# leejet/stable-diffusion.cpp

Hardware: AMD Instinct MI355X
Metric: denoise it/s (image-iterations/s: cond+uncond UNet forwards per image per step) (higher is better)
Workload: dtype f16; 1 GPU; sd15 UNet 512x512, cfg 7 (cond+uncond), f16 weights, batch 8/GPU, Euler-A step; global_batch=8, flash_attn=True, hip_graph=1, cfg_pair_in_one_graph=True, device_resident_sampler=True

## Files before the change

### stable-diffusion.cpp_amd/csrc/backend/planner.cpp

```cpp
#include "planner.h"

#include <atomic>
#include <cstddef>
#include <cstdio>
#include <cstdlib>
#include <cstring>
#include <functional>
#include <memory>
#include <mutex>
#include <string>
#include <algorithm>
#include <map>
#include <unordered_map>
#include <unordered_set>
#include <vector>

#include "kernels.h"
#include "ktime.h"

namespace mi355x {

static uint8_t g_opmap[256];
static uint8_t g_unmap[256];
static bool g_opmap_init = [] {
// ... 4268 lines not shown

namespace {
struct OptionRow {
    const char* key;
    std::atomic<int> Options::*member;
    void (*setter)(int);
};
#define OPT(name) {#name, &Options::name, nullptr}
const OptionRow g_option_table[] = {
    OPT(fusion),
    OPT(mfma_gemm),
    OPT(hip_graph),
    OPT(flash_pattern),
    {"gemm16_t320", nullptr, gemm16_set_t320},
    {"t256p_pad", nullptr, gemm16_set_t256p_pad},
    {"tail_split", nullptr, gemm16_set_tail_split},
    {"conv_wmajor", nullptr, gemm16_set_conv_wmajor},
    {"ln16_rows", nullptr, gemm16_set_ln16_rows},
    {"t320_linear_max_split", nullptr, gemm16_set_t320_linear_max_split},
    OPT(qgemv),
    OPT(fuse_q16),
    {"streamk", nullptr, gemm16_set_streamk},
    {"geglu16", nullptr, gemm16_set_geglu16},
    {"bn64_max_tiles", nullptr, gemm16_set_bn64_max},
    {"conv3w_prio", nullptr, conv3w_set_prio},
    {"t256p_min_nt_sk", nullptr, gemm16_set_t256p_min_nt_sk},
    {"t256p_min_tiles_sk", nullptr, gemm16_set_t256p_min_tiles_sk},
    {"conv3w", nullptr, conv3w_set},
    OPT(hoist_emb),
    OPT(fuse_rows16),
    OPT(fuse_cat_rows16),
    OPT(fuse_gn_stats),
    OPT(fuse_gn_epilogue),
    OPT(fuse_tile_merge),
    OPT(fuse_model_input),
    OPT(fuse_guidance3),
    OPT(fuse_patch_embed),
    OPT(fuse_ip_attn),
    OPT(fuse_joint_qkv),
    OPT(fuse_ln_reduce),
    OPT(jit_qimages),
    {"qinloop_min_rows", nullptr, gemm16_set_qinloop_min_rows},
    OPT(fuse_flash_slices),
    {"gemm16_t192p", nullptr, gemm16_set_t192p},
    {"conv3w_min_blocks", nullptr, conv3w_set_min_blocks},
    {"conv3w_min_blocks_deep", nullptr, conv3w_set_min_blocks_deep},
// ... 63 lines not shown
```

### stable-diffusion.cpp_amd/csrc/kernels/conv3w.hip

```cpp
#include <cstdio>
#include <cstdlib>

#include "device_utils.h"
#include "g16_common.h"
#include "kernels.h"
#include "ktime.h"

namespace mi355x {

template <int TW, int BN>
struct C3Geom {
    static constexpr int TR     = 256 / TW;
    static constexpr int PITCH  = TW + 16;
    static constexpr int WROWS  = TR + 2;
    static constexpr int WBYTES = WROWS * PITCH * 64;
    static constexpr int NWP    = WBYTES / 1024;
    static constexpr int NWPW   = (NWP + 7) / 8;
    static constexpr int WBUF   = NWPW * 8 * 1024;
    static constexpr int CB     = BN / 64;
    static constexpr int NF     = (BN / 32) * 2;
    static constexpr int BSTAGE = NF * 1024;
    static constexpr int NST    = 4;
    static constexpr int LDS    = 2 * WBUF + NST * BSTAGE;
    static constexpr int RB1    = TW >= 64 ? 32 * 64 : (32 / TW) * PITCH * 64;
    static_assert(WBYTES % 1024 == 0 && PITCH % 16 == 0 && NWPW <= 5 && LDS <= 160 * 1024, "window geometry");
};

#define C3_RD(DST_, ADDR_, OFF_) asm volatile("ds_read_b128 %0, %1 offset:%2" : "=v"(DST_) : "v"(ADDR_), "n"(OFF_))
#define C3_TIE(X_) asm volatile("" : "+v"(X_))

template <int TW, int BN, int PRIO = 3>
__global__ __launch_bounds__(512, 2) void k_conv3w(G16Args g) {
    using G = C3Geom<TW, BN>;
    constexpr int CB = G::CB, CL = CB - 2, PITCH = G::PITCH, NWPW = G::NWPW, WBUF = G::WBUF, BSTAGE = G::BSTAGE, NF = G::NF, RB1 = G::RB1;
    static_assert(CB >= 3, "at least three column blocks per wave");
    __shared__ __attribute__((aligned(1024))) char smem[G::LDS];

    const int lane = threadIdx.x & 63;
    const int wave = __builtin_amdgcn_readfirstlane(threadIdx.x >> 6);
    const int wr = wave & 3, wc = wave >> 2;
    const int hi = lane >> 5;
    if constexpr (PRIO == 3) {
        if (wave >= 4) __builtin_amdgcn_s_setprio(1);
    }

    int bid, kslice;
    g16_wg_order(g, g.ncol_tiles, bid, kslice);
    const int row_tile = bid / g.ncol_tiles;
    const int col_tile = bid - row_tile * g.ncol_tiles;
    const int64_t row0 = (int64_t)row_tile * 256;
    const int col0     = col_tile * BN;

    int icb0 = 0, nicb = g.nt;
    if (g.split_k > 1) {
        icb0 = kslice * g.nt_slice;
        nicb = min(g.nt_slice, g.nt - icb0);
        g.dst += (int64_t)kslice * g.slab;
    }
// ... 180 lines not shown
        C3_RD(BL[0], bcur, (0 * 2) * 1024);                                                                                  \
        C3_RD(BL[1], bcur, (1 * 2) * 1024);                                                                                  \
        if constexpr (CL > 2) C3_RD(BL[CL - 1], bcur, (2 * 2) * 1024);                                                       \
        C3_RD(BH0[0], bcur, ((CB - 2) * 2) * 1024);                                                                          \
        C3_RD(BH0[1], bcur, ((CB - 1) * 2) * 1024);                                                                          \
        for (int ib_ = 0; ib_ + 1 < nicb; ++ib_) C3_BLOCK(NP_, false);                                                       \
        C3_BLOCK(NP_, true);                                                                                                 \
        asm volatile("s_waitcnt lgkmcnt(0)" ::: "memory");                                                                   \
    } while (0)

    if constexpr (NF % 8 != 0) {
        if (w_short)
            C3_MAIN(NPBMAX - 1);
        else
            C3_MAIN(NPBMAX);
    } else {
        C3_MAIN(NPBMAX);
    }

    if (g.ep.gn_rec) {
        static_assert(4 * BN * (int)sizeof(GnRec) <= WBUF, "the tile's records fit one window buffer");
        GnRec* lds = (GnRec*)(smem + (wb ^ 1) * WBUF);
        if (g.ep.residual)
            epi_conv_gn<true, BN, 4, 2, CB>(acc, g, row0, col0, wr, wc, lane, lds);
        else
            epi_conv_gn<false, BN, 4, 2, CB>(acc, g, row0, col0, wr, wc, lane, lds);
        return;
    }
    if (g.ep.residual)
        epi_conv<1>(acc, g, row0, col0, wr, wc, lane);
    else
        epi_conv<0>(acc, g, row0, col0, wr, wc, lane);
}

static int g_conv3w_prio = 3;
void conv3w_set_prio(int v) { g_conv3w_prio = v; }
static int g_conv3w = 1;
void conv3w_set(int v) { g_conv3w = v; }
static int g_conv3w_min_blocks = 8, g_conv3w_min_blocks_deep = 5;
void conv3w_set_min_blocks(int v) { g_conv3w_min_blocks = v > 0 ? v : 1; }
void conv3w_set_min_blocks_deep(int v) { g_conv3w_min_blocks_deep = v > 0 ? v : 1; }

int conv3w_plan(int64_t W, int64_t H, int64_t IC, int64_t N, int64_t OC, int ksize, int stride, bool upscale2x, int* bn_out) {
    if (!g_conv3w || ksize != 3 || stride != 1 || upscale2x) return 0;
    if (!(W == 16 || W == 32 || W == 64 || W == 128) || (H * W) % 256 != 0 || IC < 64) return 0;
    if (N * H * W * ((IC + 63) / 64 * 64) * 2 >= (1ll << 32)) return 0;
    const int bn = OC % 320 == 0 ? 320 : (OC % 256 == 0 ? 256 : 0);
    if (!bn) return 0;
    const int64_t tiles = (H * W * N / 256) * (OC / bn);
    const int64_t nicb  = (IC + 63) / 64 * 2;
// ... 39 lines not shown
    }
    if (e.act >= 0) {
        fprintf(stderr, "ggml-mi355x: conv3w has no fused activation\n");
        abort();
    }
    G16Args g{};
    g.A    = (const _Float16*)x16_nhwc;
    g.W    = (const half8_t*)wswz32;
    g.ICp  = (int)((IC + 63) / 64 * 64);
    g.kfr  = (int64_t)g.ICp * 9 / 16;
    g.dst  = dst;
    g.H    = (int)H;
    g.Wd   = (int)W;
    g.OW   = (int)W;
    g.OH   = (int)H;
    g.OHOW = W * H;
    g.S    = 1;
    g.pad  = 1;
    g.KS   = 3;
    g.nt   = g.ICp / 32;
    g.R    = g.OHOW * N;
    g.C    = OC;
    g.zero = gemm16_zero_page();
    g.ep   = G16Epi{e.bias, e.residual, e.scale};
    g.ep.chan_add = e.chan_add;
    g.ep.chan_ld  = (int)e.chan_ld;
    g.ncol_tiles  = (int)(OC / bn);
    if (e.gn_rec) {
        if ((S > 1 && splitk_ws) || !conv3w_gn_rec_supported(g.OHOW, OC, N)) {
            fprintf(stderr, "ggml-mi355x: conv3w asked for a GroupNorm side band on a launch it does not serve (split %d, %lld positions per image)\n", S, (long long)g.OHOW);
            abort();
        }
        g.ep.gn_rec = e.gn_rec;
    }
    if (S > 1 && splitk_ws) {
        g.split_k  = S;
        g.nt_slice = (g.nt + S - 1) / S;
        g.slab     = g.R * OC;
        g.dst      = splitk_ws;
        g.ep       = G16Epi{nullptr, nullptr, e.scale};
    } else {
        S = 1;
    }
    const unsigned tiles = (unsigned)((g.R / 256) * g.ncol_tiles);
    g.worder             = gemm16_worder_rows(g, tiles, (unsigned)S);
    const double bytes   = (double)N * H * W * g.ICp * 2.0 + (double)g.ICp * 9 * ((OC + 127) / 128 * 128) * 2.0 + (double)g.R * OC * 4.0 * (e.residual ? 2.0 : 1.0);
// ... 19 lines not shown
```

### stable-diffusion.cpp_amd/csrc/kernels/g16_common.h

```cpp
#pragma once
#include "device_utils.h"
#include "kernels.h"

namespace mi355x {

struct G16Epi {
    const float* bias;
    const float* residual;
    float scale;
    const float* gate = nullptr;
    int gate_L        = 0;
    int gelu          = 0;
    const float* chan_add = nullptr;
    int chan_ld           = 0;
    GnRec* gn_rec         = nullptr;
};

__device__ __forceinline__ void gn_merge(float& m, float& q, float m2, float q2, float hn) {
    const float d = m2 - m;
    q             = (q + q2) + (d * d) * hn;
    m             = 0.5f * (m + m2);
}
template <int CTRL>
__device__ __forceinline__ float gn_dpp(float v) { return __int_as_float(__builtin_amdgcn_update_dpp(0, __float_as_int(v), CTRL, 0xf, 0xf, true)); }
// ... 55 lines not shown
    int a_runL, a_runS;
    int qt;
    int64_t qrow_bytes;
    int wblk_lim;
    int nt;
    int ncol_tiles;
    int split_k;
    int nt_slice;
    int64_t slab;
    float* sk_slab;
    int* sk_cnt;
    int sk_grid, sk_tiles, sk_dp;
    int split_col;
    _Float16* split_dst16;
    int64_t split_ldd16;
    int multi;
    const half8_t* Wm[16];
    float* dstm[16];
    _Float16* dst16m[16];
    const float* biasm[16];
    int H, Wd, ICp, OH, OW, S, pad, UPS, KS, icb_per_tap, tap_major;
    int64_t OHOW;
    const _Float16* zero;
    G16Epi ep;
#ifdef MI355X_EXPERIMENTS
    int abl;
#endif
};

int gemm16_worder_rows(const G16Args& g, unsigned gx, unsigned ny);
void gemm16_set_conv_wmajor(int v);
__device__ __forceinline__ void g16_wg_order(const G16Args& g, int ncol_all, int& bid, int& kslice) {
    if (g.worder > 0) {
        const int L  = (int)blockIdx.y * (int)gridDim.x + (int)blockIdx.x;
        const int k  = L & 7, j = L >> 3;
        const int pl = j / g.worder, r = j - pl * g.worder;
        const int p  = pl * 8 + k;
        kslice       = p / ncol_all;
        bid          = r * ncol_all + (p - kslice * ncol_all);
        return;
    }
    const int nb = gridDim.x;
    bid          = blockIdx.x;
    if ((nb & 7) == 0) bid = (bid & 7) * (nb >> 3) + (bid >> 3);
    kslice = blockIdx.y;
}

#define GLDS16(gptr, ldsptr) \
    __builtin_amdgcn_global_load_lds((const __attribute__((address_space(1))) void*)(gptr), (__attribute__((address_space(3))) void*)(ldsptr), 16, 0, 0)


template <typename T>
__device__ __forceinline__ void st_u(T* ubase, uint32_t lane_bytes, T v) { *(T*)((char*)ubase + lane_bytes) = v; }
template <typename T>
// ... 169 lines not shown
                    const int64_t uo  = ub + (int64_t)ro * g.hm_d;
                    const uint32_t lo = le + (ro >= wrap_at ? adj : 0u);
                    const float v     = acc[rb][cb][r] * g.ep.scale + bias;
                    if (MODE == EPI_HM_F32)
                        st_u(g.dst + uo, lo * 4u, v);
                    else
                        st_u(g.dst16 + uo, lo * 2u, (_Float16)v);
                }
            } else {
#pragma unroll
                for (int r = 0; r < 16; ++r) {
                    const int64_t row = base_row + (r & 3) + 8 * (r >> 2) + 4 * hi;
                    if (row >= g.R) continue;
                    float v = acc[rb][cb][r] * g.ep.scale + bias;
                    if (g.ep.residual) v += g.ep.residual[row * g.ldd + col];
                    if (g.dst) g.dst[row * g.ldd + col] = v;
                    if (g.dst16) g.dst16[row * g.ldd16 + col] = (_Float16)v;
                }
            }
        }
    }
}

template <int BM, int RB, int CB>
__device__ __forceinline__ void epi_dispatch_linear(const float16_t (&acc)[RB][CB], const G16Args& g, int64_t row0, int col0, int wr, int wc, int lane) {
    const bool full = row0 + BM <= g.R;
    if (g.geglu_inner > 0 && g.geglu16) {
        epi_geglu16(acc, g, row0, col0, wr, wc, lane);
    } else if (CB % 2 == 0 && g.geglu_inner > 0) {
        if constexpr (CB % 2 == 0) epi_geglu(acc, g, row0, col0, wr, wc, lane);
    } else if (g.hm_d > 0 && g.hm_L >= 32 && !g.ep.residual && (g.dst != nullptr) != (g.dst16 != nullptr)) {
        if (g.dst16)
            epi_linear<EPI_HM_F16>(acc, g, row0, col0, wr, wc, lane);
        else
            epi_linear<EPI_HM_F32>(acc, g, row0, col0, wr, wc, lane);
    } else if (g.ep.gate) {
        epi_linear<EPI_F32_GATE>(acc, g, row0, col0, wr, wc, lane);
    } else if (full && g.hm_d == 0 && g.dst && !g.dst16) {
        if (g.ep.residual)
            epi_linear<EPI_F32_RES>(acc, g, row0, col0, wr, wc, lane);
        else
            epi_linear<EPI_F32>(acc, g, row0, col0, wr, wc, lane);
    } else if (g.hm_d == 0 && g.dst16 && !g.dst && g.ep.residual && !g.ep.gelu) {
        epi_linear<EPI_F16_RES>(acc, g, row0, col0, wr, wc, lane);
    } else if (g.hm_d == 0 && g.dst16 && !g.dst && !g.ep.residual) {
        if (g.ep.gelu)
            epi_linear<EPI_F16_GELU>(acc, g, row0, col0, wr, wc, lane);
        else
            epi_linear<EPI_F16>(acc, g, row0, col0, wr, wc, lane);
// ... 29 lines not shown
            const float* pc  = g.ep.chan_add ? g.ep.chan_add + (int64_t)img0 * cld + cblk : nullptr;
#pragma unroll
            for (int r0 = 0; r0 < 16; r0 += 8) {
                float bv[8], rv[8];
#pragma unroll
                for (int r = r0; r < r0 + 8; ++r) {
                    const int ro  = (r & 3) + 8 * (r >> 2);
                    const bool ok = MODE != 2 || cblk + ro + 4 * hi < g.C;
                    bv[r - r0]    = (pb && ok) ? ld_u(pb + ro, 16u * hi) : 0.f;
                    if (pc && ok) bv[r - r0] += ld_u(pc + ro, (4u * hi + dimg * cld) * 4u);
                    rv[r - r0]    = ((MODE == 1 || (MODE == 2 && g.ep.residual)) && ok) ? ld_u(g.ep.residual + ub + (int64_t)ro * g.OHOW, le * 4u) : 0.f;
                }
#pragma unroll
                for (int r = r0; r < r0 + 8; ++r) {
                    const int ro = (r & 3) + 8 * (r >> 2);
                    if (MODE == 2 && cblk + ro + 4 * hi >= g.C) continue;
                    st_u(g.dst + ub + (int64_t)ro * g.OHOW, le * 4u, acc[rb][cb][r] * g.ep.scale + bv[r - r0] + rv[r - r0]);
                }
            }
        }
    }
}

template <bool RES, int BN, int WR, int RB, int CB>
__device__ __forceinline__ void epi_conv_gn(const float16_t (&acc)[RB][CB], const G16Args& g, int64_t row0, int col0, int wr, int wc, int lane, GnRec* lds) {
    static_assert(WR * RB == 8 && (RB == 1 || RB == 2), "a 256-position tile");
    const int hi = lane >> 5, lc = lane & 31;
    const uint32_t ohow = (uint32_t)g.OHOW;
    const uint32_t img0 = (uint32_t)(row0 / g.OHOW), p0 = (uint32_t)(row0 - (int64_t)img0 * g.OHOW);
    const uint32_t le   = (uint32_t)(wr * (RB * 32) + lc) + 4u * hi * ohow;
    const uint32_t cld  = g.ep.chan_ld ? (uint32_t)g.ep.chan_ld : (uint32_t)g.C;
    const int chl = gn_lane_chan(lane);
#pragma unroll
    for (int cb = 0; cb < CB; ++cb) {
        const int cblk   = col0 + (wc * CB + cb) * 32;
        const int64_t ub = ((int64_t)img0 * g.C + cblk) * g.OHOW + p0;
        const float* pb  = g.ep.bias ? g.ep.bias + cblk : nullptr;
        const float* pc  = g.ep.chan_add ? g.ep.chan_add + (int64_t)img0 * cld + cblk : nullptr;
        float v[RB][16];
#pragma unroll
        for (int r0 = 0; r0 < 16; r0 += 8) {
            float bv[8], rv[RB][8];
#pragma unroll
            for (int r = r0; r < r0 + 8; ++r) {
                const int ro = (r & 3) + 8 * (r >> 2);
                bv[r - r0]   = pb ? ld_u(pb + ro, 16u * hi) : 0.f;
                if (pc) bv[r - r0] += ld_u(pc + ro, 16u * hi);
#pragma unroll
                for (int rb = 0; rb < RB; ++rb) rv[rb][r - r0] = RES ? ld_u(g.ep.residual + ub + (int64_t)ro * g.OHOW + rb * 32, le * 4u) : 0.f;
            }
#pragma unroll
            for (int r = r0; r < r0 + 8; ++r) {
                const int ro = (r & 3) + 8 * (r >> 2);
#pragma unroll
                for (int rb = 0; rb < RB; ++rb) {
                    v[rb][r] = acc[rb][cb][r] * g.ep.scale + bv[r - r0] + rv[rb][r - r0];
                    st_u(g.dst + ub + (int64_t)ro * g.OHOW + rb * 32, le * 4u, v[rb][r]);
                }
            }
        }
        float m, q;
        gn_wave_stats<RB>(v, lane, m, q);
        if (!(lane & 1)) lds[wr * BN + (wc * CB + cb) * 32 + chl] = GnRec{m, q};
    }
    __syncthreads();
    const int c = (wc * WR + wr) * 64 + lane;
    if (c < BN) {
        GnRec a[WR];
#pragma unroll
        for (int i = 0; i < WR; ++i) a[i] = lds[i * BN + c];
        float hn = 16.f * RB;
#pragma unroll
        for (int st = 1; st < WR; st *= 2, hn *= 2.f)
#pragma unroll
            for (int i = 0; i < WR; i += 2 * st) gn_merge(a[i].mean, a[i].m2, a[i + st].mean, a[i + st].m2, hn);
        const uint32_t chunks = ohow / (uint32_t)GN_REC_CHUNK, t = p0 / (uint32_t)GN_REC_CHUNK;
        g.ep.gn_rec[((int64_t)img0 * chunks + t) * g.C + col0 + c] = a[0];
    }
}

}
```

### stable-diffusion.cpp_amd/csrc/kernels/gemm16.hip

```cpp
#include <atomic>
#include <cstdio>
#include <cstdlib>
#include <mutex>
#include <type_traits>
#include <utility>
#include <vector>
#include "device_utils.h"
#include "kernels.h"
#include "ktime.h"
#include "g16_common.h"

namespace mi355x {

template <int BM, int BN, bool CONV, int BK, int NST, int WR, int WC, int PIPE = 0, bool SK = false, int QT = 0>
__global__ __launch_bounds__(WR * WC * 64, PIPE ? 2 : 2) void k_gemm16(G16Args g) {
    static_assert(!SK || (PIPE == 1 && !CONV), "stream-K is written for the pipelined Linear tiles");
    static_assert(QT == 0 || ((QT == 8 || QT == 4) && PIPE == 1 && !CONV && !SK && BM == 256 && (BN == 256 || BN == 192) && WR * WC == 8), "in-loop dequantisation: pipelined 256 x 256 / 256 x 192 Linear tiles");
    constexpr int NW  = WR * WC;
    constexpr int RB  = BM / WR / 32;
    constexpr int CB  = BN / WC / 32;
    static_assert(RB * WR * 32 == BM && CB * WC * 32 == BN, "tile must split into 32x32 blocks per wave");
    constexpr int ROWB   = BK * 2;
    constexpr int SLOTS  = ROWB / 16;
    constexpr int RPP    = 1024 / ROWB;
// ... 2 lines not shown
    constexpr int NF     = (BN / 32) * KSTEPS;
    constexpr int APW    = (ABYTES / 1024) / NW;
    constexpr int WPW    = (NF + NW - 1) / NW;
    constexpr int WEXTRA = NF % NW;
    constexpr int BBYTES = NF * 1024;
    constexpr int NPT    = APW + WPW;
    static_assert(APW * NW * 1024 == ABYTES && APW >= 1, "A stage must split evenly over the waves");
    constexpr int QBLK  = QT == 8 ? 34 : 18;
    constexpr int QPB   = QT == 8 ? 64 : 32;
    constexpr int QNP   = QPB / 16;
    constexpr int QTOFF = 2 * QBLK - 16;
    constexpr int QVC   = 256;
    constexpr int QRAWB = QVC * (QPB + 16);
    constexpr int QNRAW = 3;
    constexpr int QPI   = QT ? QVC * QNP / (NW * 64) : 0;
    constexpr int QRQ   = QPI + 1;
    constexpr int QB0   = NST * ABYTES;
    constexpr int QR0   = QB0 + 2 * BBYTES;
    constexpr int SMEMB = QT ? QR0 + QNRAW * QRAWB : NST * (ABYTES + BBYTES);
    static_assert(SMEMB <= 160 * 1024, "LDS budget");
    __shared__ __attribute__((aligned(1024))) char smem[SMEMB];
    constexpr bool G16_GN_REC_TILE = CONV && BM == 256 && BN != 128 && ((WR == 4 && RB == 2) || (WR == 8 && RB == 1));
    static_assert(!G16_GN_REC_TILE || WR * BN * (int)sizeof(GnRec) <= SMEMB, "the tile's records fit the staging ring");

    const int lane0 = threadIdx.x & 63;
    const int wave = __builtin_amdgcn_readfirstlane(threadIdx.x >> 6);
    const int wr = wave % WR, wc = wave / WR;

    int64_t sk_u = 0, sk_end = 0;
    int sk_w = 0;
    int dp_t = 0, dp_end = 0;
    if constexpr (SK) {
        const int64_t U = (int64_t)(g.sk_tiles - g.sk_dp) * g.nt;
        sk_w            = (g.sk_grid & 7) == 0 ? (int)(blockIdx.x & 7) * (g.sk_grid >> 3) + (int)(blockIdx.x >> 3) : (int)blockIdx.x;
        sk_u            = (int64_t)sk_w * U / g.sk_grid;
        sk_end          = (int64_t)(sk_w + 1) * U / g.sk_grid;
        const int per   = g.sk_dp / g.sk_grid;
        dp_t            = sk_w * per;
        dp_end          = dp_t + per;
    }
  for (bool sk_more = true; sk_more;) {
    int lane = lane0;
    if constexpr (SK) asm volatile("" : "+v"(lane));
    int bid = blockIdx.x, kslice = blockIdx.y;
    int kt0 = 0, nt = g.nt;
    if constexpr (SK) {
// ... 773 lines not shown
                for (int rb = 0; rb < RB; ++rb)
#pragma unroll
                    for (int cb = 0; cb < CB; ++cb)
#pragma unroll
                        for (int i4 = 0; i4 < 4; ++i4) {
                            const u32x4_t v = __builtin_amdgcn_raw_buffer_load_b128(rp, ((((wave * RB + rb) * CB + cb) * 4 + i4) * 64 + lane) * 16, 0, 16);
                            acc[rb][cb][4 * i4] += __uint_as_float(v[0]);
                            acc[rb][cb][4 * i4 + 1] += __uint_as_float(v[1]);
                            acc[rb][cb][4 * i4 + 2] += __uint_as_float(v[2]);
                            acc[rb][cb][4 * i4 + 3] += __uint_as_float(v[3]);
                        }
            }
        }
    }

    if (!CONV) {
        if (PIPE == 1 && BN == 256 && g.split_col > 0) {
            const bool hi_part = col0 >= g.split_col;
            G16Args gs   = g;
            gs.dst       = hi_part ? nullptr : g.dst;
            gs.dst16     = hi_part ? g.split_dst16 : nullptr;
            gs.ldd16     = hi_part ? g.split_ldd16 : 0;
            gs.ep.gelu   = hi_part ? 1 : 0;
            epi_dispatch_linear<BM>(acc, gs, row0, col0, wr, wc, lane);
        } else
        epi_dispatch_linear<BM>(acc, g, row0, col0, wr, wc, lane);
    } else if (G16_GN_REC_TILE && g.ep.gn_rec) {
        if constexpr (G16_GN_REC_TILE) {
            __syncthreads();
            if (g.ep.residual)
                epi_conv_gn<true, BN, WR, RB, CB>(acc, g, row0, col0, wr, wc, lane, (GnRec*)smem);
            else
                epi_conv_gn<false, BN, WR, RB, CB>(acc, g, row0, col0, wr, wc, lane, (GnRec*)smem);
        }
    } else {
        const bool fullc = col0 + BN <= g.C;
        if (fullc) {
            if (g.ep.residual)
                epi_conv<1>(acc, g, row0, col0, wr, wc, lane);
            else
                epi_conv<0>(acc, g, row0, col0, wr, wc, lane);
        } else {
            epi_conv<2>(acc, g, row0, col0, wr, wc, lane);
        }
    }
  }
}

static inline int64_t rup64(int64_t a, int64_t b) { return (a + b - 1) / b * b; }

static int g_g16_variant = 3;
static int g_g16_tap_major = 0;
void gemm16_set_tap_major(int v) { g_g16_tap_major = v; }
int gemm16_tap_major() { return g_g16_tap_major; }
void gemm16_set_variant(int v) { g_g16_variant = v; }
static inline bool g16_bk32() { return g_g16_variant == 1 || g_g16_variant == 3; }

enum { G16_T128 = 0, G16_T256 = 1, G16_T256W = 2, G16_T160 = 3, G16_T160N = 4, G16_T320 = 5, G16_T256P = 6, G16_T128N64 = 7, G16_T192P = 8 };
static int g_g16_force_tile = -1;
void gemm16_set_tile(int t) { g_g16_force_tile = t; }
// ... 119 lines not shown
    if (!g_g16_geglu16 || g_g16_variant != 3 || !g16_bk32() || g_g16_force_tile >= 0 || (M / 2) % 16 != 0) return 1;
    const int tile = g16_pick_tile(rows, M, 2, false, 0, rup64(K, 64) / 32, 1);
    return (tile == G16_T160 || tile == G16_T160N || tile == G16_T320) ? 2 : 1;
}
static int g_g16_qinloop_min_rows = 513;
void gemm16_set_qinloop_min_rows(int v) { g_g16_qinloop_min_rows = v; }
bool gemm16_qinloop_supported(int wtype, int64_t rows, int64_t M, int64_t K, int mul, int split) {
    if (g_g16_qinloop_min_rows <= 0 || rows < g_g16_qinloop_min_rows || (wtype != 8 && wtype != 2)) return false;
    if (g_g16_variant != 3 || !g16_bk32() || g_g16_force_tile >= 0 || g_g16_streamk) return false;
    if (K % 64 != 0 || K < 192 || g16_use_bn64(rows, M, mul)) return false;
    const int64_t nt = K / 32;
    if (split > 1 || gemm16_split_k(rows, M, K, false) > 1) return false;
    const int tile = g16_pick_tile(rows, M, 0, false, 0, nt, mul);
    return (tile == G16_T256P || tile == G16_T192P) && M % 64 == 0;
}
bool gemm16_split_col_supported(int64_t rows, int64_t M, int64_t K) {
    if (g_g16_variant != 3 || !g16_bk32() || M % 256 != 0 || M % 160 == 0 || g16_use_bn64(rows, M, 1)) return false;
    const int64_t nt = rup64(K, 64) / 32;
    return gemm16_split_k(rows, M, K, false) == 1 && g16_pick_tile(rows, M, false, false, 0, nt, 1) == G16_T256P;
}

static int g_g16_conv_wmajor = 1;
void gemm16_set_conv_wmajor(int v) { g_g16_conv_wmajor = v; }
int gemm16_worder_rows(const G16Args& g, unsigned gx, unsigned ny) {
    if (!g_g16_conv_wmajor || g.KS == 0 || g.ncol_tiles <= 0 || g.multi > 1 || g.sk_grid > 0) return 0;
    if (gx % 8 != 0 || gx % (unsigned)g.ncol_tiles != 0 || ((unsigned)g.ncol_tiles * ny) % 8 != 0) return 0;
    const int nrow = (int)(gx / (unsigned)g.ncol_tiles);
    if (nrow < 2) return 0;
    const int64_t imgs = g.OHOW > 0 ? g.R / g.OHOW : 1;
    const double act   = (double)imgs * g.H * g.Wd * g.ICp * 2.0;
    const double wts   = (double)g.ICp * g.KS * g.KS * (double)rup64(g.C, 128) * 2.0;
    return wts >= 2.0 * act ? nrow : 0;
}
static bool g16_trace();
static std::atomic<int64_t> g_conv_route_launches[CONV_ROUTE_COUNT];
void conv_route_taken(ConvRoute r) { g_conv_route_launches[r].fetch_add(1, std::memory_order_relaxed); }
int64_t conv_route_launches(int route) { return route >= 0 && route < CONV_ROUTE_COUNT ? g_conv_route_launches[route].load(std::memory_order_relaxed) : 0; }
static std::atomic<int64_t> g_linear_route_launches[LIN_ROUTE_COUNT];
void linear_route_taken(LinearRoute r) { g_linear_route_launches[r].fetch_add(1, std::memory_order_relaxed); }
int64_t linear_route_launches(int route) { return route >= 0 && route < LIN_ROUTE_COUNT ? g_linear_route_launches[route].load(std::memory_order_relaxed) : 0; }
static bool g16_gn_rec_tile_ok(int tile, int64_t C, int64_t ohow, int ny) {
    const int bn = (tile == G16_T160 || tile == G16_T160N) ? 160 : (tile == G16_T320 ? 320 : (tile == G16_T256P ? 256 : 0));
    return bn > 0 && ny == 1 && C % bn == 0 && ohow % GN_REC_CHUNK == 0;
}
[[noreturn]] static void g16_gn_rec_contract_violation() {
    fprintf(stderr, "ggml-mi355x: conv launch asked for a GroupNorm side band on a shape / tile it does not serve\n");
    abort();
}
template <int BN_, bool CONV_>
static void g16_launch(hipStream_t s, G16Args& g, int64_t rows, double flops, double bytes) {
    const unsigned ny = g.split_k > 1 ? (unsigned)g.split_k : 1u;
    const int mul     = (!CONV_ && g.multi > 1) ? g.multi : 1;
    if (BN_ == 128 && g_g16_variant == 3 && (!g.sk_cnt || g.sk_grid > 0)) {
        const int tile = g16_pick_tile(rows, g.C, g.geglu_inner > 0 ? (g.geglu16 ? 2 : 1) : 0, CONV_, g.split_k > 1 ? g.split_k : 0, g.nt, mul);
        if (g16_trace()) fprintf(stderr, "G16 tile %d rows=%lld C=%lld nt=%d split=%d mul=%d qt=%d\n", tile, (long long)rows, (long long)g.C, g.nt, g.split_k, mul, g.qt);
        if (g.qt && ((tile != G16_T256P && tile != G16_T192P) || g.sk_grid > 0 || g.C % 64 != 0 || g.nt < 6 || (g.nt & 1) || (g.split_k > 1 && ((g.nt_slice & 1) || g.nt_slice < 6 || g.nt - (g.split_k - 1) * g.nt_slice < 6)))) {
            fprintf(stderr, "ggml-mi355x: in-loop dequantisation planned for a launch that does not take the pipelined 256 x 256 tile (tile %d, rows %lld, M %lld, K stages %d)\n", tile, (long long)rows, (long long)g.C, g.nt);
            abort();
        }
        if (g.geglu_inner > 0 && g.geglu16 && tile != G16_T160 && tile != G16_T160N && tile != G16_T320) {
            fprintf(stderr, "ggml-mi355x: GEGLU launch planned on the 16-column interleave, but its tile takes the paired image\n");
            abort();
        }
        if constexpr (!CONV_) {
            if (g.sk_grid > 0) {
                KScope ks_(s, KF_LINEAR, flops, bytes);
                if (tile == G16_T256P) {
                    linear_route_taken(LIN_STREAMK);
                    g.ncol_tiles = (int)((g.C + 255) / 256);
                    k_gemm16<256, 256, false, 32, 4, 4, 2, 1, true><<<dim3((unsigned)g.sk_grid, 1), 512, 0, s>>>(g);
                } else {
                    fprintf(stderr, "ggml-mi355x: stream-K launch planned for a shape that does not take a pipelined tile\n");
                    abort();
// ... 1414 lines not shown
```

### stable-diffusion.cpp_amd/csrc/kernels/kernels.h

```cpp
#pragma once
#include <hip/hip_runtime.h>
#include <stddef.h>
#include <stdint.h>

namespace mi355x {

struct View4 {
    const void* data;
    int64_t ne[4];
    int64_t nb[4];
    int type;
};

enum BinOp { BIN_ADD = 0, BIN_SUB = 1, BIN_MUL = 2, BIN_DIV = 3 };
enum UnOp { UN_SILU = 0, UN_GELU = 1, UN_GELU_QUICK = 2, UN_SIGMOID = 3, UN_TANH = 4, UN_RELU = 5, UN_NEG = 6, UN_EXP = 7, UN_GELU_ERF = 8 };

enum EwRoute {
    EW_BIN_SAME = 0, EW_BIN_ROWVEC, EW_BIN_TOKVEC, EW_BIN_CHAN, EW_BIN_GENERIC,
    EW_COPY_CONTIG, EW_COPY_TRANSPOSE, EW_COPY_ROWS, EW_COPY_GENERIC,
    EW_CONCAT_DIM2, EW_CONCAT_PLANES, EW_CONCAT_GENERIC,
    EW_TILE_MERGE_V4, EW_TILE_MERGE_V1,
    EW_ROUTE_COUNT
};
int64_t elementwise_route_launches(int route);
// ... 108 lines not shown
int gemm16_tap_major();
void gemm16_set_splitk_target(int v);
void gemm16_set_splitk_mid(int v);
void gemm16_set_tile(int t);
#ifdef MI355X_EXPERIMENTS
void gemm16_set_abl(int v);
#endif
void gemm16_set_t320(int v);
void gemm16_set_t256p_pad(int v);
void gemm16_set_conv_wmajor(int v);
void gemm16_set_ln16_rows(int v);
void gemm16_set_tail_split(int v);
void gemm16_set_bn64(int v);
void gemm16_set_variant(int v);
void launch_gemm16_linear(hipStream_t s, float* dst, void* dst16, int64_t ldd16, const void* a16, int64_t lda, const void* wswz, int64_t rows,
                          int64_t K, int64_t M, int64_t ldd, const Epilogue& ep, int hm_d = 0, int hm_H = 0, int hm_L = 0, float* splitk_ws = nullptr, int* splitk_cnt = nullptr, int splitk_S = 0);
void launch_gemm16_linear_multi(hipStream_t s, int n, float* const* dst, void* const* dst16, const void* a16, int64_t lda, const void* const* wswz, int64_t rows,
                               int64_t K, int64_t M, const float* const* bias, float scale, int hm_d, int hm_H, int hm_L);
void launch_gemm16_linear_geglu(hipStream_t s, void* dst16, const void* a16, int64_t lda, const void* wswz_geglu, int64_t rows, int64_t K, int64_t M,
                                const float* bias, float* splitk_ws = nullptr, int* splitk_cnt = nullptr, int splitk_S = 0, int geglu_mode = 1);
int gemm16_geglu_mode(int64_t rows, int64_t M, int64_t K);
void gemm16_set_bn64_max(int v);
void gemm16_set_geglu16(int v);
int gemm16_split_k(int64_t rows, int64_t M, int64_t K, bool conv);
bool splitk_reduce_gn_supported(int64_t hw, int64_t C, int64_t N, int groups);
bool splitk_reduce_ln_supported(int64_t rows, int64_t M);
void gemm16_set_t320_linear_max_split(int v);
struct G16SplitPlan {
    int S;
    bool inkernel;
    size_t ws_bytes;
    int tiles;
};
G16SplitPlan gemm16_split_plan(int64_t rows, int64_t M, int64_t K, bool conv, bool plain_out, bool geglu = false);
void gemm16_set_splitk_inkernel(int v);
void gemm16_set_splitk_in_target(int v);
void launch_gemm16_conv(hipStream_t s, float* dst, const void* x16_nhwc, const void* wswz, int64_t W, int64_t H, int64_t IC, int64_t N, int64_t OC,
                        int ksize, int stride, int pad, bool upscale2x, const Epilogue& ep, float* splitk_ws = nullptr, int* splitk_cnt = nullptr, int splitk_S = 0);
bool gemm16_conv_gn_rec_supported(int64_t OHOW, int64_t N, int64_t OC, int64_t ICp, int ksize);
enum ConvRoute {
    CONV_C3W_TW16_BN256 = 0, CONV_C3W_TW16_BN320, CONV_C3W_TW32_BN256, CONV_C3W_TW32_BN320, CONV_C3W_TW64_BN256, CONV_C3W_TW64_BN320, CONV_C3W_TW128_BN256, CONV_C3W_TW128_BN320,
    CONV_G16_T128, CONV_G16_T128N64, CONV_G16_T256, CONV_G16_T256W, CONV_G16_T160, CONV_G16_T160N, CONV_G16_T320, CONV_G16_T256P,
    CONV_SPLITK_REDUCE,
    CONV_WMAJOR,
    CONV_ROUTE_COUNT
};
// ... 96 lines not shown
```

Measured before the change: 379.3 it/s.

## Software-pipeline GEMM and conv epilogue loads ahead of stores

Adds pipelined epilogue variants for the linear, conv and GroupNorm-record paths. They issue the bias, channel-add and residual loads for upcoming 8-row batches before storing the current batch, so global-load latency overlaps with the stores. Pipeline depth and warm-up are chosen at compile time per tile shape, and some high-occupancy tiles are excluded to limit register pressure. The feature is on by default behind a runtime option; the extra live registers could cut occupancy or cause spills.

```diff
diff --git a/stable-diffusion.cpp_amd/csrc/backend/planner.cpp b/stable-diffusion.cpp_amd/csrc/backend/planner.cpp
--- a/stable-diffusion.cpp_amd/csrc/backend/planner.cpp
+++ b/stable-diffusion.cpp_amd/csrc/backend/planner.cpp
@@ -4314,6 +4314,7 @@
     OPT(fuse_q16),
     {"streamk", nullptr, gemm16_set_streamk},
     {"geglu16", nullptr, gemm16_set_geglu16},
+    {"epi_pipeline", nullptr, gemm16_set_epi_pipeline},
     {"bn64_max_tiles", nullptr, gemm16_set_bn64_max},
     {"conv3w_prio", nullptr, conv3w_set_prio},
     {"t256p_min_nt_sk", nullptr, gemm16_set_t256p_min_nt_sk},
diff --git a/stable-diffusion.cpp_amd/csrc/kernels/conv3w.hip b/stable-diffusion.cpp_amd/csrc/kernels/conv3w.hip
--- a/stable-diffusion.cpp_amd/csrc/kernels/conv3w.hip
+++ b/stable-diffusion.cpp_amd/csrc/kernels/conv3w.hip
@@ -34,6 +34,7 @@
     using G = C3Geom<TW, BN>;
     constexpr int CB = G::CB, CL = CB - 2, PITCH = G::PITCH, NWPW = G::NWPW, WBUF = G::WBUF, BSTAGE = G::BSTAGE, NF = G::NF, RB1 = G::RB1;
     static_assert(CB >= 3, "at least three column blocks per wave");
+    constexpr int C3_EPI_DEPTH = 1, C3_EPI_WARM = BN == 320 ? 4 : 0, C3_EPI_GN = BN == 320 ? 0 : 1;
     __shared__ __attribute__((aligned(1024))) char smem[G::LDS];
 
     const int lane = threadIdx.x & 63;
@@ -260,10 +261,19 @@
         static_assert(4 * BN * (int)sizeof(GnRec) <= WBUF, "the tile's records fit one window buffer");
         GnRec* lds = (GnRec*)(smem + (wb ^ 1) * WBUF);
         if (g.ep.residual)
-            epi_conv_gn<true, BN, 4, 2, CB>(acc, g, row0, col0, wr, wc, lane, lds);
+            epi_conv_gn<true, BN, 4, C3_EPI_GN>(acc, g, row0, col0, wr, wc, lane, lds);
         else
-            epi_conv_gn<false, BN, 4, 2, CB>(acc, g, row0, col0, wr, wc, lane, lds);
+            epi_conv_gn<false, BN, 4, C3_EPI_GN>(acc, g, row0, col0, wr, wc, lane, lds);
         return;
+    }
+    if constexpr (C3_EPI_DEPTH > 0) {
+        if (g.epi_pipe) {
+            if (g.ep.residual)
+                epi_conv_pipe<1, C3_EPI_DEPTH, C3_EPI_WARM>(acc, g, row0, col0, wr, wc, lane);
+            else
+                epi_conv_pipe<0, C3_EPI_DEPTH, C3_EPI_WARM>(acc, g, row0, col0, wr, wc, lane);
+            return;
+        }
     }
     if (g.ep.residual)
         epi_conv<1>(acc, g, row0, col0, wr, wc, lane);
@@ -349,6 +359,7 @@
     g.R    = g.OHOW * N;
     g.C    = OC;
     g.zero = gemm16_zero_page();
+    g.epi_pipe = gemm16_epi_pipeline();
     g.ep   = G16Epi{e.bias, e.residual, e.scale};
     g.ep.chan_add = e.chan_add;
     g.ep.chan_ld  = (int)e.chan_ld;
diff --git a/stable-diffusion.cpp_amd/csrc/kernels/g16_common.h b/stable-diffusion.cpp_amd/csrc/kernels/g16_common.h
--- a/stable-diffusion.cpp_amd/csrc/kernels/g16_common.h
+++ b/stable-diffusion.cpp_amd/csrc/kernels/g16_common.h
@@ -1,4 +1,7 @@
 #pragma once
+#include <type_traits>
+#include <utility>
+
 #include "device_utils.h"
 #include "kernels.h"
 
@@ -101,6 +104,7 @@
     int H, Wd, ICp, OH, OW, S, pad, UPS, KS, icb_per_tap, tap_major;
     int64_t OHOW;
     const _Float16* zero;
+    int epi_pipe;
     G16Epi ep;
 #ifdef MI355X_EXPERIMENTS
     int abl;
@@ -109,6 +113,7 @@
 
 int gemm16_worder_rows(const G16Args& g, unsigned gx, unsigned ny);
 void gemm16_set_conv_wmajor(int v);
+int gemm16_epi_pipeline();
 __device__ __forceinline__ void g16_wg_order(const G16Args& g, int ncol_all, int& bid, int& kslice) {
     if (g.worder > 0) {
         const int L  = (int)blockIdx.y * (int)gridDim.x + (int)blockIdx.x;
@@ -324,9 +329,106 @@
     }
 }
 
-template <int BM, int RB, int CB>
+template <int... I, class F>
+__device__ __forceinline__ void epi_static_for(std::integer_sequence<int, I...>, F&& f) {
+    (f(std::integral_constant<int, I>{}), ...);
+}
+constexpr int epi_issued(int i, int NB, int DEPTH, int WARM) { return i < 0 ? -1 : (i < WARM ? i : (i + DEPTH < NB ? i + DEPTH : NB - 1)); }
+template <int NB, int DEPTH, int WARM, class LD, class ST>
+__device__ __forceinline__ void epi_pipe_run(LD&& load, ST&& store) {
+    epi_static_for(std::make_integer_sequence<int, NB>{}, [&](auto ic) __attribute__((always_inline)) {
+        constexpr int i = decltype(ic)::value, lo = epi_issued(i - 1, NB, DEPTH, WARM) + 1, hi = epi_issued(i, NB, DEPTH, WARM);
+        epi_static_for(std::make_integer_sequence<int, hi - lo + 1>{}, [&](auto jc) __attribute__((always_inline)) { load(std::integral_constant<int, lo + decltype(jc)::value>{}); });
+        store(ic);
+    });
+}
+
+template <int MODE, int DEPTH, int RB, int CB>
+__device__ __forceinline__ void epi_linear_pipe(const float16_t (&acc)[RB][CB], const G16Args& g, int64_t row0, int col0, int wr, int wc, int lane) {
+    static_assert(MODE == EPI_F32_RES || MODE == EPI_F16_RES || MODE == EPI_F32_GATE, "the Linear variants that load per element");
+    static_assert(DEPTH >= 1, "at least one batch in flight");
+    constexpr int NB = RB * CB * 2, NBUF = DEPTH + 1;
+    const int hi = lane >> 5, lc = lane & 31;
+    const uint32_t lr = (uint32_t)(lc + 4 * hi * (int)g.ldd) * 4u;
+    const uint32_t lb16 = (uint32_t)(lc + 4 * hi * (int)g.ldd16) * 2u;
+    float rv[NBUF][8], bias[NBUF], g0[NBUF], g1[NBUF];
+    auto load = [&](auto bc) __attribute__((always_inline)) {
+        constexpr int bl = decltype(bc)::value, rb = bl / (2 * CB), cb = (bl >> 1) % CB, r0 = (bl & 1) * 8, s = bl % NBUF, sp = (bl + NBUF - 1) % NBUF;
+        const int64_t base_row = row0 + wr * (RB * 32) + rb * 32;
+        const int cblk = col0 + (wc * CB + cb) * 32, col = cblk + lc;
+        const bool okc = col < g.C;
+        if constexpr (r0 == 0) {
+            bias[s] = 0.f;
+            if (MODE == EPI_F32_GATE) g0[s] = g1[s] = 0.f;
+        } else {
+            bias[s] = bias[sp];
+            if (MODE == EPI_F32_GATE) g0[s] = g0[sp], g1[s] = g1[sp];
+        }
+#pragma unroll
+        for (int j = 0; j < 8; ++j) rv[s][j] = 0.f;
+        if (!okc || (MODE != EPI_F32_RES && base_row >= g.R)) return;
+        if constexpr (r0 == 0) {
+            if (g.ep.bias) bias[s] = g.ep.bias[col];
+            if (MODE == EPI_F32_GATE) {
+                const uint32_t n0 = (uint32_t)base_row / (uint32_t)g.ep.gate_L;
+                g0[s] = g.ep.gate[(int64_t)n0 * g.C + col];
+                if ((int64_t)(n0 + 1) * g.ep.gate_L < g.R) g1[s] = g.ep.gate[(int64_t)(n0 + 1) * g.C + col];
+            }
+        }
+        const float* ur = g.ep.residual + base_row * g.ldd + cblk;
+        if (MODE == EPI_F32_RES || base_row + 32 <= g.R) {
+#pragma unroll
+            for (int r = r0; r < r0 + 8; ++r) rv[s][r - r0] = ld_u(ur + (int64_t)((r & 3) + 8 * (r >> 2)) * g.ldd, lr);
+        } else {
+            const int nvl = (int)(g.R - base_row) - 4 * hi;
+#pragma unroll
+            for (int r = r0; r < r0 + 8; ++r) {
+                const int ro = (r & 3) + 8 * (r >> 2);
+                if (ro < nvl) rv[s][r - r0] = ld_u(ur + (int64_t)ro * g.ldd, lr);
+            }
+        }
+    };
+    auto store = [&](auto bc) __attribute__((always_inline)) {
+        constexpr int i = decltype(bc)::value, rb = i / (2 * CB), cb = (i >> 1) % CB, r0 = (i & 1) * 8, s = i % NBUF;
+        const int64_t base_row = row0 + wr * (RB * 32) + rb * 32;
+        const int cblk = col0 + (wc * CB + cb) * 32, col = cblk + lc;
+        if (col >= g.C) return;
+        const int nvl = MODE == EPI_F32_RES ? 32 : (int)(g.R - base_row < 32 ? g.R - base_row : 32) - 4 * hi;
+        int wrap_at = 0;
+        if (MODE == EPI_F32_GATE) {
+            const uint32_t n0 = (uint32_t)base_row / (uint32_t)g.ep.gate_L, l0 = (uint32_t)base_row - n0 * (uint32_t)g.ep.gate_L;
+            wrap_at = g.ep.gate_L - (int)l0 - 4 * hi;
+        }
+        float* ub      = MODE == EPI_F16_RES ? nullptr : g.dst + base_row * g.ldd + cblk;
+        _Float16* ub16 = MODE == EPI_F16_RES ? g.dst16 + base_row * g.ldd16 + cblk : nullptr;
+#pragma unroll
+        for (int r = r0; r < r0 + 8; ++r) {
+            const int ro = (r & 3) + 8 * (r >> 2);
+            if (ro >= nvl) continue;
+            if (MODE == EPI_F32_RES)
+                st_u(ub + (int64_t)ro * g.ldd, lr, acc[rb][cb][r] * g.ep.scale + bias[s] + rv[s][r - r0]);
+            else if (MODE == EPI_F16_RES)
+                st_u(ub16 + (int64_t)ro * g.ldd16, lb16, (_Float16)(acc[rb][cb][r] * g.ep.scale + bias[s] + rv[s][r - r0]));
+            else
+                st_u(ub + (int64_t)ro * g.ldd, lr, (acc[rb][cb][r] * g.ep.scale + bias[s]) * (ro >= wrap_at ? g1[s] : g0[s]) + rv[s][r - r0]);
+        }
+    };
+    epi_pipe_run<NB, DEPTH, 0>(load, store);
+}
+
+template <int BM, int EPD, int RB, int CB>
 __device__ __forceinline__ void epi_dispatch_linear(const float16_t (&acc)[RB][CB], const G16Args& g, int64_t row0, int col0, int wr, int wc, int lane) {
     const bool full = row0 + BM <= g.R;
+    if constexpr (EPD > 0) {
+        if (g.epi_pipe && !(g.geglu_inner > 0) && !(g.hm_d > 0 && g.hm_L >= 32 && !g.ep.residual && (g.dst != nullptr) != (g.dst16 != nullptr))) {
+            if (g.ep.gate) return epi_linear_pipe<EPI_F32_GATE, EPD>(acc, g, row0, col0, wr, wc, lane);
+            if (full && g.hm_d == 0 && g.dst && !g.dst16) {
+                if (g.ep.residual) return epi_linear_pipe<EPI_F32_RES, EPD>(acc, g, row0, col0, wr, wc, lane);
+            } else if (g.hm_d == 0 && g.dst16 && !g.dst && g.ep.residual && !g.ep.gelu) {
+                return epi_linear_pipe<EPI_F16_RES, EPD>(acc, g, row0, col0, wr, wc, lane);
+            }
+        }
+    }
     if (g.geglu_inner > 0 && g.geglu16) {
         epi_geglu16(acc, g, row0, col0, wr, wc, lane);
     } else if (CB % 2 == 0 && g.geglu_inner > 0) {
@@ -402,7 +504,83 @@
     }
 }
 
-template <bool RES, int BN, int WR, int RB, int CB>
+template <int MODE, int DEPTH, int WARM, int RB, int CB>
+__device__ __forceinline__ void epi_conv_pipe(const float16_t (&acc)[RB][CB], const G16Args& g, int64_t row0, int col0, int wr, int wc, int lane) {
+    static_assert(DEPTH >= 1, "at least one batch in flight");
+    constexpr int NB = RB * CB * 2, NBUF = DEPTH + 1;
+    constexpr bool RES = MODE == 1 || MODE == 2;
+    const int hi = lane >> 5, lc = lane & 31;
+    const uint32_t ohow = (uint32_t)g.OHOW;
+    const uint32_t cld  = g.ep.chan_ld ? (uint32_t)g.ep.chan_ld : (uint32_t)g.C;
+    const float* res    = RES ? g.ep.residual : nullptr;
+    uint32_t img0[RB], le[RB], dimg[RB];
+    bool okr[RB];
+#pragma unroll
+    for (int rb = 0; rb < RB; ++rb) {
+        const int64_t pos_base = row0 + wr * (RB * 32) + rb * 32;
+        okr[rb]  = pos_base + lc < g.R;
+        img0[rb] = (uint32_t)(pos_base < g.R ? pos_base : 0) / ohow;
+        const uint32_t p0 = (uint32_t)(pos_base < g.R ? pos_base : 0) - img0[rb] * ohow;
+        uint32_t pl = p0 + lc, di = 0;
+        while (pl >= ohow) {
+            pl -= ohow;
+            ++di;
+        }
+        dimg[rb] = di;
+        le[rb]   = di * (uint32_t)g.C * ohow + pl + 4u * hi * ohow;
+    }
+    float bq[NBUF][8], cq[NBUF][8], rq[NBUF][8];
+    auto load = [&](auto bc) __attribute__((always_inline)) {
+        constexpr int bl = decltype(bc)::value, rb = bl / (2 * CB), cb = (bl >> 1) % CB, r0 = (bl & 1) * 8, s = bl % NBUF;
+        const int cblk = col0 + (wc * CB + cb) * 32;
+#pragma unroll
+        for (int j = 0; j < 8; ++j) bq[s][j] = cq[s][j] = rq[s][j] = 0.f;
+        if (!(okr[rb] && cblk < g.C)) return;
+        const int64_t ub = ((int64_t)img0[rb] * g.C + cblk) * g.OHOW;
+        const float* pb  = g.ep.bias ? g.ep.bias + cblk : nullptr;
+        const float* pc  = g.ep.chan_add ? g.ep.chan_add + (int64_t)img0[rb] * cld + cblk : nullptr;
+        if (MODE != 2) {
+            if (pb) {
+#pragma unroll
+                for (int r = r0; r < r0 + 8; ++r) bq[s][r - r0] = ld_u(pb + (r & 3) + 8 * (r >> 2), 16u * hi);
+            }
+            if (pc) {
+#pragma unroll
+                for (int r = r0; r < r0 + 8; ++r) cq[s][r - r0] = ld_u(pc + (r & 3) + 8 * (r >> 2), (4u * hi + dimg[rb] * cld) * 4u);
+            }
+            if (res) {
+#pragma unroll
+                for (int r = r0; r < r0 + 8; ++r) rq[s][r - r0] = ld_u(res + ub + (int64_t)((r & 3) + 8 * (r >> 2)) * g.OHOW, le[rb] * 4u);
+            }
+        } else {
+#pragma unroll
+            for (int r = r0; r < r0 + 8; ++r) {
+                const int ro = (r & 3) + 8 * (r >> 2);
+                if (cblk + ro + 4 * hi >= g.C) continue;
+                if (pb) bq[s][r - r0] = ld_u(pb + ro, 16u * hi);
+                if (pc) cq[s][r - r0] = ld_u(pc + ro, (4u * hi + dimg[rb] * cld) * 4u);
+                if (res) rq[s][r - r0] = ld_u(res + ub + (int64_t)ro * g.OHOW, le[rb] * 4u);
+            }
+        }
+    };
+    auto store = [&](auto bc) __attribute__((always_inline)) {
+        constexpr int i = decltype(bc)::value, rb = i / (2 * CB), cb = (i >> 1) % CB, r0 = (i & 1) * 8, s = i % NBUF;
+        const int cblk = col0 + (wc * CB + cb) * 32;
+        if (!(okr[rb] && cblk < g.C)) return;
+        const int64_t ub = ((int64_t)img0[rb] * g.C + cblk) * g.OHOW;
+#pragma unroll
+        for (int r = r0; r < r0 + 8; ++r) {
+            const int ro = (r & 3) + 8 * (r >> 2);
+            if (MODE == 2 && cblk + ro + 4 * hi >= g.C) continue;
+            float bv = bq[s][r - r0];
+            if (g.ep.chan_add) bv += cq[s][r - r0];
+            st_u(g.dst + ub + (int64_t)ro * g.OHOW, le[rb] * 4u, acc[rb][cb][r] * g.ep.scale + bv + rq[s][r - r0]);
+        }
+    };
+    epi_pipe_run<NB, DEPTH, WARM>(load, store);
+}
+
+template <bool RES, int BN, int WR, int DEPTH, int RB, int CB>
 __device__ __forceinline__ void epi_conv_gn(const float16_t (&acc)[RB][CB], const G16Args& g, int64_t row0, int col0, int wr, int wc, int lane, GnRec* lds) {
     static_assert(WR * RB == 8 && (RB == 1 || RB == 2), "a 256-position tile");
     const int hi = lane >> 5, lc = lane & 31;
@@ -411,6 +589,62 @@
     const uint32_t le   = (uint32_t)(wr * (RB * 32) + lc) + 4u * hi * ohow;
     const uint32_t cld  = g.ep.chan_ld ? (uint32_t)g.ep.chan_ld : (uint32_t)g.C;
     const int chl = gn_lane_chan(lane);
+    bool piped = false;
+    if constexpr (DEPTH > 0) {
+        piped = g.epi_pipe != 0;
+        if (piped) {
+            constexpr int NB = CB * 2, NBUF = DEPTH + 1;
+            float bq[NBUF][8], cq[NBUF][8], rq[NBUF][RB][8], v[RB][16];
+#pragma unroll
+            for (int i = -DEPTH; i < NB; ++i) {
+                const int bl = i + DEPTH;
+                if (bl < NB) {
+                    const int cb = bl >> 1, r0 = (bl & 1) * 8, s = bl % NBUF;
+                    const int cblk   = col0 + (wc * CB + cb) * 32;
+                    const int64_t ub = ((int64_t)img0 * g.C + cblk) * g.OHOW + p0;
+                    const float* pb  = g.ep.bias ? g.ep.bias + cblk : nullptr;
+                    const float* pc  = g.ep.chan_add ? g.ep.chan_add + (int64_t)img0 * cld + cblk : nullptr;
+#pragma unroll
+                    for (int j = 0; j < 8; ++j) bq[s][j] = cq[s][j] = 0.f;
+                    if (pb) {
+#pragma unroll
+                        for (int r = r0; r < r0 + 8; ++r) bq[s][r - r0] = ld_u(pb + (r & 3) + 8 * (r >> 2), 16u * hi);
+                    }
+                    if (pc) {
+#pragma unroll
+                        for (int r = r0; r < r0 + 8; ++r) cq[s][r - r0] = ld_u(pc + (r & 3) + 8 * (r >> 2), 16u * hi);
+                    }
+#pragma unroll
+                    for (int r = r0; r < r0 + 8; ++r)
+#pragma unroll
+                        for (int rb = 0; rb < RB; ++rb)
+                            rq[s][rb][r - r0] = RES ? ld_u(g.ep.residual + ub + (int64_t)((r & 3) + 8 * (r >> 2)) * g.OHOW + rb * 32, le * 4u) : 0.f;
+                }
+                if (i >= 0) {
+                    const int cb = i >> 1, r0 = (i & 1) * 8, s = i % NBUF;
+                    const int cblk   = col0 + (wc * CB + cb) * 32;
+                    const int64_t ub = ((int64_t)img0 * g.C + cblk) * g.OHOW + p0;
+#pragma unroll
+                    for (int r = r0; r < r0 + 8; ++r) {
+                        const int ro = (r & 3) + 8 * (r >> 2);
+                        float bv = bq[s][r - r0];
+                        if (g.ep.chan_add) bv += cq[s][r - r0];
+#pragma unroll
+                        for (int rb = 0; rb < RB; ++rb) {
+                            v[rb][r] = acc[rb][cb][r] * g.ep.scale + bv + rq[s][rb][r - r0];
+                            st_u(g.dst + ub + (int64_t)ro * g.OHOW + rb * 32, le * 4u, v[rb][r]);
+                        }
+                    }
+                    if (r0 == 8) {
+                        float m, q;
+                        gn_wave_stats<RB>(v, lane, m, q);
+                        if (!(lane & 1)) lds[wr * BN + (wc * CB + cb) * 32 + chl] = GnRec{m, q};
+                    }
+                }
+            }
+        }
+    }
+    if (!piped) {
 #pragma unroll
     for (int cb = 0; cb < CB; ++cb) {
         const int cblk   = col0 + (wc * CB + cb) * 32;
@@ -443,6 +677,7 @@
         gn_wave_stats<RB>(v, lane, m, q);
         if (!(lane & 1)) lds[wr * BN + (wc * CB + cb) * 32 + chl] = GnRec{m, q};
     }
+    }
     __syncthreads();
     const int c = (wc * WR + wr) * 64 + lane;
     if (c < BN) {
diff --git a/stable-diffusion.cpp_amd/csrc/kernels/gemm16.hip b/stable-diffusion.cpp_amd/csrc/kernels/gemm16.hip
--- a/stable-diffusion.cpp_amd/csrc/kernels/gemm16.hip
+++ b/stable-diffusion.cpp_amd/csrc/kernels/gemm16.hip
@@ -48,6 +48,13 @@
     __shared__ __attribute__((aligned(1024))) char smem[SMEMB];
     constexpr bool G16_GN_REC_TILE = CONV && BM == 256 && BN != 128 && ((WR == 4 && RB == 2) || (WR == 8 && RB == 1));
     static_assert(!G16_GN_REC_TILE || WR * BN * (int)sizeof(GnRec) <= SMEMB, "the tile's records fit the staging ring");
+    constexpr bool G16_EPI_160ACC = BM == 256 && (BN == 320 || (BN == 160 && WR == 4));
+    constexpr bool G16_EPI_OCC4   = BM == 256 && BN == 128 && WR == 4;
+    constexpr bool G16_EPI_OCC3   = BM == 256 && BN == 160 && WR == 8;
+    constexpr int G16_EPI_LIN  = G16_EPI_OCC4 ? 0 : ((BM == 256 && (BN == 256 || G16_EPI_OCC3)) ? 1 : 2);
+    constexpr int G16_EPI_CONV = (G16_EPI_OCC4 || G16_EPI_OCC3) ? 0 : 1;
+    constexpr int G16_EPI_WARM = G16_EPI_160ACC ? 4 : 0;
+    constexpr int G16_EPI_GN   = (G16_EPI_160ACC || G16_EPI_OCC3) ? 0 : 1;
 
     const int lane0 = threadIdx.x & 63;
     const int wave = __builtin_amdgcn_readfirstlane(threadIdx.x >> 6);
@@ -867,20 +874,27 @@
             gs.dst16     = hi_part ? g.split_dst16 : nullptr;
             gs.ldd16     = hi_part ? g.split_ldd16 : 0;
             gs.ep.gelu   = hi_part ? 1 : 0;
-            epi_dispatch_linear<BM>(acc, gs, row0, col0, wr, wc, lane);
+            epi_dispatch_linear<BM, G16_EPI_LIN>(acc, gs, row0, col0, wr, wc, lane);
         } else
-        epi_dispatch_linear<BM>(acc, g, row0, col0, wr, wc, lane);
+        epi_dispatch_linear<BM, G16_EPI_LIN>(acc, g, row0, col0, wr, wc, lane);
     } else if (G16_GN_REC_TILE && g.ep.gn_rec) {
         if constexpr (G16_GN_REC_TILE) {
             __syncthreads();
             if (g.ep.residual)
-                epi_conv_gn<true, BN, WR, RB, CB>(acc, g, row0, col0, wr, wc, lane, (GnRec*)smem);
+                epi_conv_gn<true, BN, WR, G16_EPI_GN>(acc, g, row0, col0, wr, wc, lane, (GnRec*)smem);
             else
-                epi_conv_gn<false, BN, WR, RB, CB>(acc, g, row0, col0, wr, wc, lane, (GnRec*)smem);
+                epi_conv_gn<false, BN, WR, G16_EPI_GN>(acc, g, row0, col0, wr, wc, lane, (GnRec*)smem);
         }
     } else {
         const bool fullc = col0 + BN <= g.C;
-        if (fullc) {
+        if (G16_EPI_CONV > 0 && g.epi_pipe) {
+            if (!fullc)
+                epi_conv_pipe<2, G16_EPI_CONV ? G16_EPI_CONV : 1, G16_EPI_WARM>(acc, g, row0, col0, wr, wc, lane);
+            else if (g.ep.residual)
+                epi_conv_pipe<1, G16_EPI_CONV ? G16_EPI_CONV : 1, G16_EPI_WARM>(acc, g, row0, col0, wr, wc, lane);
+            else
+                epi_conv_pipe<0, G16_EPI_CONV ? G16_EPI_CONV : 1, G16_EPI_WARM>(acc, g, row0, col0, wr, wc, lane);
+        } else if (fullc) {
             if (g.ep.residual)
                 epi_conv<1>(acc, g, row0, col0, wr, wc, lane);
             else
@@ -1046,6 +1060,9 @@
 
 static int g_g16_conv_wmajor = 1;
 void gemm16_set_conv_wmajor(int v) { g_g16_conv_wmajor = v; }
+static int g_g16_epi_pipeline = 1;
+void gemm16_set_epi_pipeline(int v) { g_g16_epi_pipeline = v; }
+int gemm16_epi_pipeline() { return g_g16_epi_pipeline; }
 int gemm16_worder_rows(const G16Args& g, unsigned gx, unsigned ny) {
     if (!g_g16_conv_wmajor || g.KS == 0 || g.ncol_tiles <= 0 || g.multi > 1 || g.sk_grid > 0) return 0;
     if (gx % 8 != 0 || gx % (unsigned)g.ncol_tiles != 0 || ((unsigned)g.ncol_tiles * ny) % 8 != 0) return 0;
@@ -1073,6 +1090,7 @@
 }
 template <int BN_, bool CONV_>
 static void g16_launch(hipStream_t s, G16Args& g, int64_t rows, double flops, double bytes) {
+    g.epi_pipe        = g_g16_epi_pipeline;
     const unsigned ny = g.split_k > 1 ? (unsigned)g.split_k : 1u;
     const int mul     = (!CONV_ && g.multi > 1) ? g.multi : 1;
     if (BN_ == 128 && g_g16_variant == 3 && (!g.sk_cnt || g.sk_grid > 0)) {
diff --git a/stable-diffusion.cpp_amd/csrc/kernels/kernels.h b/stable-diffusion.cpp_amd/csrc/kernels/kernels.h
--- a/stable-diffusion.cpp_amd/csrc/kernels/kernels.h
+++ b/stable-diffusion.cpp_amd/csrc/kernels/kernels.h
@@ -154,6 +154,7 @@
 int gemm16_geglu_mode(int64_t rows, int64_t M, int64_t K);
 void gemm16_set_bn64_max(int v);
 void gemm16_set_geglu16(int v);
+void gemm16_set_epi_pipeline(int v);
 int gemm16_split_k(int64_t rows, int64_t M, int64_t K, bool conv);
 bool splitk_reduce_gn_supported(int64_t hw, int64_t C, int64_t N, int groups);
 bool splitk_reduce_ln_supported(int64_t rows, int64_t M);
```

Result: no change. 378.0 it/s (-0.3%).
